# UWQuickstep/quickstep

Hardware: AMD Instinct MI355X
Metric: probe+aggregate rows/s at TPC-H SF100 (Q1,Q3) (higher is better)
Workload: dtype i32 keys / f64 sums

## Files before the change

### quickstep_amd/csrc/join.hip

```cpp

#include "common.hpp"
#include "join_dense.hpp"
#include "join_lds.hpp"
#include "scan.hpp"

#include <atomic>
#include <cstdlib>
#include <vector>
#include <mutex>
#include <shared_mutex>
#include <type_traits>

namespace qsx {

constexpr int kJBlock = 256;
constexpr uint64_t kEmpty64 = ~0ull;
constexpr uint32_t kEmptyTid = 0xFFFFFFFFu;

struct alignas(16) LongEntry {
  int64_t key;
  uint32_t tid;
  uint32_t pad;
};

// ... 1086 lines not shown
  if (rc_control != QSX_OK) return rc_control;
  t->reserved = 0;
  t->max_tid.store(-1);
  t->seal_state.store(0);
  t->scanned.store(false);
  drop_cover(t);
  mark_stream(t, as_stream(stream));
  return QSX_OK;
}

int qsx_join_table_size(qsx_join_table_t *t, int64_t *out_entries, qsx_stream_t stream) {
  QSX_REQUIRE_DEVICE();
  if (t == nullptr || out_entries == nullptr) return QSX_ERR_INVALID_ARGUMENT;
  unsigned long long v[kControlWords] = {0, 0, 0, 0, 0, 0};
  const int rc_words = copy_control_words(t->entries_dev, as_stream(stream), v);
  if (rc_words != QSX_OK) return rc_words;
  *out_entries = static_cast<int64_t>(v[0]);
  if (t->dense && static_cast<int>(v[3] & 0xFFFFFFFFu) != 0) return QSX_ERR_INVALID_ARGUMENT;
  return QSX_OK;
}

int qsx_join_build(qsx_join_table_t *t, const void *keys_dev, int64_t n, int32_t base_tid,
                   const uint64_t *filter_dev, qsx_stream_t stream) {
  QSX_REQUIRE_DEVICE();
  if (t == nullptr || n < 0 || base_tid < 0) return QSX_ERR_INVALID_ARGUMENT;
  if (n == 0) return QSX_OK;
  if (keys_dev == nullptr) return QSX_ERR_INVALID_ARGUMENT;
  if (static_cast<int64_t>(base_tid) + n > INT32_MAX) return QSX_ERR_INVALID_ARGUMENT;
  int rc = ensure_room(t, n);
  if (rc != QSX_OK) return rc;
  t->seal_state.store(0);
  t->scanned.store(false);
  drop_cover(t);
  for (int64_t seen = t->max_tid.load(); seen < base_tid + n - 1 && !t->max_tid.compare_exchange_weak(seen, base_tid + n - 1);) {}
  std::shared_lock<std::shared_mutex> lock(t->mutex);
  const int grid = grid_for(n, kJBlock * 4);
  if (t->dense) {
    const int dgrid = grid_for((n + 63) >> 6, (kDBlock / kWave) * kBuildR);
    if (t->key_type == QSX_INT) {
      hipLaunchKernelGGL(dense_build_kernel<int32_t>, dim3(dgrid), dim3(kDBlock), 0, as_stream(stream), t->dense_view(),
                         static_cast<const int32_t *>(keys_dev), n, base_tid, filter_dev, t->entries_dev);
    } else {
      hipLaunchKernelGGL(dense_build_kernel<int64_t>, dim3(dgrid), dim3(kDBlock), 0, as_stream(stream), t->dense_view(),
                         static_cast<const int64_t *>(keys_dev), n, base_tid, filter_dev, t->entries_dev);
    }
    QSX_CHECK_LAUNCH();
    return QSX_OK;
  }
  if (t->key_type == QSX_INT) {
    hipLaunchKernelGGL(build_kernel<int32_t>, dim3(grid), dim3(kJBlock), 0, as_stream(stream), t->view(),
                       static_cast<const int32_t *>(keys_dev), n, base_tid, filter_dev, t->entries_dev);
  } else {
    hipLaunchKernelGGL(build_kernel<int64_t>, dim3(grid), dim3(kJBlock), 0, as_stream(stream), t->view(),
                       static_cast<const int64_t *>(keys_dev), n, base_tid, filter_dev, t->entries_dev);
  }
  QSX_CHECK_LAUNCH();
  mark_stream(t, as_stream(stream));
  return QSX_OK;
}

static int check_key_coding(const qsx_key_coding_t **coding, int64_t num_blocks) {
  if (*coding == nullptr) return QSX_OK;
  if ((*coding)->block_code_width == nullptr) {
    *coding = nullptr;
    return QSX_OK;
  }
  bool any = false;
  for (int64_t b = 0; b < num_blocks; ++b) {
    const int w = (*coding)->block_code_width[b];
    if (w != 0 && w != 1 && w != 2 && w != 4) return QSX_ERR_INVALID_ARGUMENT;
    if (w == 0 && (*coding)->block_dictionaries != nullptr && (*coding)->block_dictionaries[b] != nullptr) return QSX_ERR_INVALID_ARGUMENT;
    any = any || w != 0;
  }
  if (!any) *coding = nullptr;
  return QSX_OK;
}

static int join_build_blocks_impl(qsx_join_table_t *t, int64_t num_blocks, const int64_t *block_rows, const void *const *block_keys,
                          const int32_t *block_base_tids, const uint64_t *const *block_filters, const qsx_key_coding_t *coding, qsx_stream_t stream) {
  QSX_REQUIRE_DEVICE();
  if (t == nullptr || num_blocks < 0 || (num_blocks > 0 && (block_rows == nullptr || block_keys == nullptr || block_base_tids == nullptr))) {
    return QSX_ERR_INVALID_ARGUMENT;
  }
  if (check_key_coding(&coding, num_blocks) != QSX_OK) return QSX_ERR_INVALID_ARGUMENT;
  std::vector<int64_t> base(static_cast<size_t>(num_blocks));
  int64_t total = 0;
  for (int64_t b = 0; b < num_blocks; ++b) {
    if (block_rows[b] < 0 || (block_rows[b] > 0 && block_keys[b] == nullptr) || block_base_tids[b] < 0 ||
        static_cast<int64_t>(block_base_tids[b]) + block_rows[b] > INT32_MAX) {
      return QSX_ERR_INVALID_ARGUMENT;
    }
    base[b] = block_base_tids[b];
    total += block_rows[b];
  }
  if (total == 0) return QSX_OK;
  int rc = ensure_room(t, total);
  if (rc != QSX_OK) return rc;
  t->seal_state.store(0);
  t->scanned.store(false);
  drop_cover(t);
  for (int64_t b = 0; b < num_blocks; ++b) {
    const int64_t last = base[b] + block_rows[b] - 1;
    for (int64_t seen = t->max_tid.load(); seen < last && !t->max_tid.compare_exchange_weak(seen, last);) {}
  }
  hipStream_t s = as_stream(stream);
  std::vector<long long> table;
  const long long groups = build_run_table(kBuildTile, num_blocks, block_rows, block_keys,
                                           reinterpret_cast<const void *const *>(block_filters), nullptr, base.data(), &table,
                                           coding != nullptr ? coding->block_code_width : nullptr,
                                           coding != nullptr ? coding->block_dictionaries : nullptr);
  if (groups < 0) return QSX_ERR_INVALID_ARGUMENT;
  const size_t bytes = table.size() * sizeof(long long);
  const long long *runs_dev = static_cast<const long long *>(staged_device_buffer(s, bytes));
  if (runs_dev == nullptr) return QSX_ERR_OUT_OF_MEMORY;
  rc = staged_upload(s, table.data(), bytes);
  if (rc != QSX_OK) return rc;
  std::shared_lock<std::shared_mutex> lock(t->mutex);
  if (t->dense) {
    const int dgrid = grid_for(groups, kDBlock / kWave);
    if (t->key_type == QSX_INT) {
      hipLaunchKernelGGL((dense_build_kernel<int32_t, true>), dim3(dgrid), dim3(kDBlock), 0, s, t->dense_view(),
                         static_cast<const int32_t *>(nullptr), total, 0, static_cast<const uint64_t *>(nullptr), t->entries_dev, runs_dev);
    } else {
      hipLaunchKernelGGL((dense_build_kernel<int64_t, true>), dim3(dgrid), dim3(kDBlock), 0, s, t->dense_view(),
                         static_cast<const int64_t *>(nullptr), total, 0, static_cast<const uint64_t *>(nullptr), t->entries_dev, runs_dev);
    }
  } else {
    const int grid = grid_for(groups, kJBlock / kWave);
    if (t->key_type == QSX_INT) {
      hipLaunchKernelGGL(build_runs_kernel<int32_t>, dim3(grid), dim3(kJBlock), 0, s, t->view(), runs_dev, t->entries_dev);
    } else {
      hipLaunchKernelGGL(build_runs_kernel<int64_t>, dim3(grid), dim3(kJBlock), 0, s, t->view(), runs_dev, t->entries_dev);
    }
  }
  QSX_CHECK_LAUNCH();
  mark_stream(t, s);
  return QSX_OK;
}

int qsx_join_build_blocks(qsx_join_table_t *t, int64_t num_blocks, const int64_t *block_rows, const void *const *block_keys,
                          const int32_t *block_base_tids, const uint64_t *const *block_filters, qsx_stream_t stream) {
  return join_build_blocks_impl(t, num_blocks, block_rows, block_keys, block_base_tids, block_filters, nullptr, stream);
}
int qsx_join_build_blocks_coded(qsx_join_table_t *t, int64_t num_blocks, const int64_t *block_rows, const void *const *block_keys,
                                const qsx_key_coding_t *coding, const int32_t *block_base_tids, const uint64_t *const *block_filters,
                                qsx_stream_t stream) {
  return join_build_blocks_impl(t, num_blocks, block_rows, block_keys, block_base_tids, block_filters, coding, stream);
}

}

static std::atomic<long long> g_compact_probes{0};
extern "C" long long qsx_debug_join_compact_probes(void) { return g_compact_probes.load(std::memory_order_relaxed); }
static bool lds_tables_enabled() {
  const char *e = getenv("QSX_JOIN_LDS");
  return e == nullptr || e[0] != '0';
}

static bool dense_two_pass(const uint64_t *filter) {
  const char *e = getenv("QSX_JOIN_TWO_PASS");
  if (e != nullptr && e[0] != '\0') return e[0] != '0';
  return filter != nullptr;
}

static void drop_cover(qsx_join_table *t) {
  std::lock_guard<std::mutex> lock(t->cover_mutex);
  t->cover_state = 0;
  t->cover_sig.clear();
}

constexpr int64_t kAdaptiveMinRows = 1 << 16;
static bool adaptive_enabled() {
  const char *e = getenv("QSX_JOIN_ADAPTIVE");
  return e == nullptr || e[0] != '0';
}

static void sealed_pack(qsx_join_table *t, hipStream_t stream) {
  auto behind_the_pack = [&]() {
    if (t->pack_stream != stream && t->pack_event != nullptr && hipEventQuery(t->pack_event) != hipSuccess) {
      (void)hipGetLastError();
      (void)hipStreamWaitEvent(stream, t->pack_event, 0);
    }
  };
  int state = t->seal_state.load(std::memory_order_acquire);
  if (state == 2) {
    behind_the_pack();
    return;
  }
  if (state != 0 || !adaptive_enabled()) return;
  const uint64_t bytes4 = t->range * 4, bytes3 = t->range * 3;
  if (bytes4 <= (13ull << 18) || bytes3 > (36ull << 20) / 10 || t->max_tid.load() >= (1 << 23) - 2 || t->reserved >= (1 << 23) - 1) {
    return;
  }
  std::lock_guard<std::mutex> lock(t->seal_mutex);
  state = t->seal_state.load(std::memory_order_acquire);
  if (state != 0) {
    if (state == 2) behind_the_pack();
    return;
  }
  if (t->head3 == nullptr && device_malloc(&t->head3, static_cast<size_t>(bytes3) + 4) != hipSuccess) {
    (void)hipGetLastError();
    t->head3 = nullptr;
    t->seal_state.store(1, std::memory_order_release);
    return;
  }
  if (t->pack_event == nullptr && hipEventCreateWithFlags(&t->pack_event, hipEventDisableTiming) != hipSuccess) {
    (void)hipGetLastError();
    t->pack_event = nullptr;
    t->seal_state.store(1, std::memory_order_release);
    return;
  }
  hipLaunchKernelGGL(dense_pack_kernel, dim3(grid_for(static_cast<int64_t>(t->range), kJBlock * 4)), dim3(kJBlock), 0, stream, t->head, t->range,
                     t->head3);
  if (hipGetLastError() != hipSuccess || hipEventRecord(t->pack_event, stream) != hipSuccess) {
    (void)hipGetLastError();
    (void)hipStreamSynchronize(stream);
    t->seal_state.store(1, std::memory_order_release);
    return;
  }
  t->pack_stream = stream;
  t->seal_state.store(2, std::memory_order_release);
}

static bool compact_enabled() {
  const char *e = getenv("QSX_JOIN_COMPACT");
  return e == nullptr || e[0] != '0';
}
static bool compact_possible(const qsx_join_table *t) {
  const uint64_t buckets = t->capacity / kBucketSlots;
  return compact_enabled() && t->key_type == QSX_INT && buckets >= kCompactMinBuckets && buckets <= 0xFFFFFFFFull && t->max_tid.load() < (1 << 24);
}
static bool seal_compact(qsx_join_table *t, bool duplicate_keys, hipStream_t stream) {
  if (!compact_possible(t) || duplicate_keys) return false;
  if (t->compact_capacity != t->capacity) {
    (void)device_free(t->compact);
    t->compact = nullptr;
    t->compact_capacity = 0;
    if (device_malloc(&t->compact, static_cast<size_t>(t->capacity) * 5 + 16) != hipSuccess) {
      (void)hipGetLastError();
      t->compact = nullptr;
      return false;
    }
    t->compact_capacity = t->capacity;
  }
  hipLaunchKernelGGL(compact_build_kernel, dim3(static_cast<unsigned>((t->capacity + kJBlock - 1) / kJBlock)), dim3(kJBlock), 0, stream, t->view(),
                     static_cast<uint32_t *>(t->compact), static_cast<unsigned char *>(t->compact) + t->capacity * 4);
  if (hipGetLastError() != hipSuccess) return false;
  return true;
}

static bool seal_verify_enabled() {
  const char *e = getenv("QSX_JOIN_SEAL_VERIFY");
  return e != nullptr && e[0] == '1';
}
static bool wait_for_builds(qsx_join_table *t, hipStream_t stream) {
  bool marked = true;
  std::lock_guard<std::mutex> lock(t->marks_mutex);
  for (const auto &m : t->marks) {
    if (m.second == nullptr) marked = false;
    else if (m.first != stream && hipStreamWaitEvent(stream, m.second, 0) != hipSuccess) marked = false;
  }
  if (!marked) (void)hipGetLastError();
  return marked;
}
static bool read_control_words(qsx_join_table *t, hipStream_t stream, unsigned long long *v, bool *any_key) {
  if (t->control_host == nullptr && hipHostMalloc(reinterpret_cast<void **>(&t->control_host), kControlBytes, hipHostMallocDefault) != hipSuccess) {
    (void)hipGetLastError();
    t->control_host = nullptr;
  }
  if (t->control_host == nullptr) return copy_control_words(t->entries_dev, stream, v, any_key) == QSX_OK;
  if (hipMemcpyAsync(t->control_host, t->entries_dev, kControlBytes, hipMemcpyDeviceToHost, stream) != hipSuccess ||
      hipStreamSynchronize(stream) != hipSuccess) {
    return false;
  }
  *any_key = fold_control_words(t->control_host, v);
  return true;
}
static void behind_the_seal(qsx_join_table *t, hipStream_t stream) {
  if (t->seal_stream != stream && t->seal_event != nullptr && hipEventQuery(t->seal_event) != hipSuccess) {
    (void)hipGetLastError();
    (void)hipStreamWaitEvent(stream, t->seal_event, 0);
  }
}
static bool record_seal(qsx_join_table *t, hipStream_t stream) {
  if (t->seal_event == nullptr && hipEventCreateWithFlags(&t->seal_event, hipEventDisableTiming) != hipSuccess) {
    (void)hipGetLastError();
    t->seal_event = nullptr;
  }
  if (t->seal_event == nullptr || hipEventRecord(t->seal_event, stream) != hipSuccess) {
    (void)hipGetLastError();
    if (hipStreamSynchronize(stream) != hipSuccess) return false;
    t->seal_stream = nullptr;
    if (t->seal_event != nullptr) {
      (void)hipEventDestroy(t->seal_event);
      t->seal_event = nullptr;
    }
  } else {
    t->seal_stream = stream;
  }
  return true;
}
static bool publish_seal(qsx_join_table *t, hipStream_t stream, int state) {
  if (!record_seal(t, stream)) return false;
  t->seal_state.store(state, std::memory_order_release);
  return true;
}
// ... 42 lines not shown
    return nullptr;
  };
  if (!adaptive_enabled()) return stays_hashed();
  if (not_worth_a_look) {
    (void)ensure_scanned();
    return nullptr;
  }
  unsigned long long v[kControlWords];
  bool any_key = false;
  if (!put_behind_builds() || !read_control_words(t, stream, v, &any_key)) return stays_hashed();
  const uint64_t entries = v[0];
  const int64_t lo = static_cast<int64_t>(v[4] ^ 0x8000000000000000ull), hi = static_cast<int64_t>(v[5] ^ 0x8000000000000000ull);
  const uint64_t span = static_cast<uint64_t>(hi) - static_cast<uint64_t>(lo);
  const bool fits_lds = small_build && entries >= 1 && span < static_cast<uint64_t>(kLdsDenseMaxWords);
  if (!any_key || (entries < static_cast<uint64_t>(kAdaptiveMinRows) && !fits_lds) || (span >= 8 * entries && !fits_lds) ||
      span >= (1ull << 32) || entries > 0x7FFFFFFFull) {
    if (!ensure_scanned()) return nullptr;
    if (!compact_possible(t) || !read_control_words(t, stream, v, &any_key) || !seal_compact(t, v[2] != 0, stream) || !publish_seal(t, stream, 3)) {
      t->seal_state.store(1, std::memory_order_release);
    }
    return nullptr;
  }
  qsx_join_table *shadow = t->shadow;
  if (shadow != nullptr && (shadow->min_key != lo || shadow->range != span + 1 || shadow->ov_capacity < entries)) {
    (void)qsx_join_table_destroy(shadow);
    shadow = t->shadow = nullptr;
  }
  if (shadow == nullptr) {
    if (qsx_join_table_create_dense(t->key_type, lo, hi, 1, static_cast<int64_t>(entries), &shadow) != QSX_OK) {
      (void)hipGetLastError();
      return stays_hashed();
    }
    t->shadow = shadow;
  } else if (qsx_join_table_clear(shadow, reinterpret_cast<qsx_stream_t>(stream)) != QSX_OK) {
    return stays_hashed();
  }
  shadow->reserved = static_cast<int64_t>(entries);
  shadow->max_tid.store(t->max_tid.load());
  const TableView src = t->view();
  hipLaunchKernelGGL(dense_build_from_slots_kernel, dim3(grid_for(static_cast<int64_t>(src.num_slots()), kJBlock * 4)), dim3(kJBlock), 0, stream,
                     t->key_type == QSX_LONG ? 1 : 0, src, shadow->dense_view());
  if (hipGetLastError() != hipSuccess) return stays_hashed();
  if (seal_verify_enabled()) {
    int error = 0;
    if (hipStreamSynchronize(stream) != hipSuccess ||
        hipMemcpy(&error, shadow->entries_dev + 3, sizeof(error), hipMemcpyDeviceToHost) != hipSuccess || error != 0) {
      set_last_error("QSX_JOIN_SEAL_VERIFY: the shadow's build reported an error", hipErrorUnknown);
      return stays_hashed();
    }
  }
  if (!publish_seal(t, stream, 2)) return stays_hashed();
  return shadow;
}

template <int MODE, bool kRuns, bool kLds = true, int NLIP = 0>
static int launch_lds_dense_probe(qsx_join_table_t *t, const void *keys, int64_t n, int32_t probe_base_tid, const uint64_t *filter,
                                  int32_t *out_probe, int32_t *out_build, int64_t capacity, unsigned long long *count,
                                  uint64_t *out_bitmap, int anti, hipStream_t stream, const long long *runs_dev, int64_t tiles,
                                  const LipViews &lips = LipViews{}) {
  const size_t table_bytes = kLds ? ((static_cast<size_t>(t->range) * 4 + 15) & ~static_cast<size_t>(15)) : 0;
  auto launch = [&](auto key_tag) -> int {
    using KeyT = decltype(key_tag);
    auto kernel = &lds_dense_probe_kernel<KeyT, MODE, kRuns, kLds, NLIP>;
    if (table_bytes > 48 * 1024) {
      QSX_HIP_TRY(hipFuncSetAttribute(reinterpret_cast<const void *>(kernel), hipFuncAttributeMaxDynamicSharedMemorySize, 160 * 1024 - kLdsStaticBytes));
    }
    const int sub = kLds ? kLdsSub : kLdsSubGlobal, per_cu = kLds ? 1 : 2;
    const int64_t units = (tiles + sub - 1) / sub;
    const int grid = static_cast<int>(units < static_cast<int64_t>(per_cu) * kCUs ? units : static_cast<int64_t>(per_cu) * kCUs);
    hipLaunchKernelGGL(kernel, dim3(grid), dim3(kLdsBlock), table_bytes, stream, t->dense_view(), static_cast<const KeyT *>(keys), n, probe_base_tid,
                       filter, out_probe, out_build, capacity, count, out_bitmap, anti, runs_dev, lips);
    QSX_CHECK_LAUNCH();
    return QSX_OK;
  };
  return t->key_type == QSX_INT ? launch(int32_t{}) : launch(int64_t{});
}

static bool one_pass_enabled() {
  const char *e = getenv("QSX_JOIN_ONE_PASS");
  return e == nullptr || e[0] != '0';
}

template <int MODE, bool kRuns = false>
static int launch_probe(qsx_join_table_t *t, const void *keys, int64_t n, int32_t probe_base_tid,
                        const uint64_t *filter, int32_t *out_probe, int32_t *out_build,
                        int64_t capacity, int64_t *out_count, uint64_t *out_bitmap, int anti,
                        hipStream_t stream, const long long *runs_dev = nullptr, int64_t run_tiles = 0) {
  static_assert(kDenseTile == kProbeTile, "one run table serves both table kinds");
  if (!t->dense && n != 0) {
    qsx_join_table *shadow = sealed_shadow(t, stream, n);
    if (shadow != nullptr) {
      return launch_probe<MODE, kRuns>(shadow, keys, n, probe_base_tid, filter, out_probe, out_build, capacity, out_count, out_bitmap,
                                       anti, stream, runs_dev, run_tiles);
    }
    if (!t->scanned.load(std::memory_order_acquire)) {
      set_last_error("the scan in front of a hashed table's first probe could not be issued", hipErrorUnknown);
      return QSX_ERR_HIP;
    }
  }
  if (out_count != nullptr) QSX_HIP_TRY(hipMemsetAsync(out_count, 0, sizeof(int64_t), stream));
  if (n == 0) return QSX_OK;
  if (t->dense) sealed_pack(t, stream);
  std::shared_lock<std::shared_mutex> lock(t->mutex);
  if (t->dense) {
    const int64_t tiles = kRuns ? run_tiles : (n + kDenseTile - 1) / kDenseTile;
    const int64_t limit = 8 * kCUs;
    const int dgrid = static_cast<int>(tiles < limit ? tiles : limit);
    unsigned long long *dcount = reinterpret_cast<unsigned long long *>(out_count);
    if constexpr (MODE == 0 || MODE == 1 || MODE == 2) {
      const bool two_pass = MODE == 0 && dense_two_pass(filter);
      if (!two_pass && lds_tables_enabled() && t->range <= static_cast<uint64_t>(kLdsDenseMaxWords) && n >= 32 * static_cast<int64_t>(t->range) &&
          n >= (1 << 18)) {
        return launch_lds_dense_probe<MODE, kRuns>(t, keys, n, probe_base_tid, filter, out_probe, out_build, capacity, dcount, out_bitmap, anti,
                                                   stream, runs_dev, tiles);
      }
    }
    if constexpr (MODE == 0) {
      if (dense_two_pass(filter) && one_pass_enabled() && n >= (1 << 20)) {
        return launch_lds_dense_probe<0, kRuns, false>(t, keys, n, probe_base_tid, filter, out_probe, out_build, capacity, dcount, out_bitmap, anti,
                                                       stream, runs_dev, tiles);
      }
    }
    if (MODE == 0 && dense_two_pass(filter)) {
      const int64_t units = tiles * (kDBlock / kWave);
      CallScratch scratch(stream);
      const size_t bytes_counts = static_cast<size_t>(units) * 4, bytes_offsets = static_cast<size_t>(units + 1) * 8,
                   bytes_scan = scan_workspace_words(units) * 8;
      const int rc_scratch = scratch.reserve(CallScratch::padded(bytes_counts) + CallScratch::padded(bytes_offsets) + CallScratch::padded(bytes_scan));
      if (rc_scratch != QSX_OK) return rc_scratch;
      int32_t *unit_counts = static_cast<int32_t *>(scratch.take(bytes_counts));
      int64_t *unit_offsets = static_cast<int64_t *>(scratch.take(bytes_offsets)), *scan_ws = static_cast<int64_t *>(scratch.take(bytes_scan));
      if (t->key_type == QSX_INT) {
        hipLaunchKernelGGL((dense_probe_kernel<int32_t, 3, kRuns>), dim3(dgrid), dim3(kDBlock), 0, stream, t->dense_view(),
                           static_cast<const int32_t *>(keys), n, probe_base_tid, filter, out_probe, out_build, capacity,
                           dcount, out_bitmap, anti, unit_counts, unit_offsets, runs_dev);
      } else {
        hipLaunchKernelGGL((dense_probe_kernel<int64_t, 3, kRuns>), dim3(dgrid), dim3(kDBlock), 0, stream, t->dense_view(),
                           static_cast<const int64_t *>(keys), n, probe_base_tid, filter, out_probe, out_build, capacity,
                           dcount, out_bitmap, anti, unit_counts, unit_offsets, runs_dev);
      }
      QSX_CHECK_LAUNCH();
      QSX_HIP_TRY(launch_scan(unit_counts, units, unit_offsets, out_count, scan_ws, stream));
      if (t->key_type == QSX_INT) {
        hipLaunchKernelGGL((dense_probe_kernel<int32_t, 4, kRuns>), dim3(dgrid), dim3(kDBlock), 0, stream, t->dense_view(),
                           static_cast<const int32_t *>(keys), n, probe_base_tid, filter, out_probe, out_build, capacity,
                           dcount, out_bitmap, anti, unit_counts, unit_offsets, runs_dev);
      } else {
        hipLaunchKernelGGL((dense_probe_kernel<int64_t, 4, kRuns>), dim3(dgrid), dim3(kDBlock), 0, stream, t->dense_view(),
                           static_cast<const int64_t *>(keys), n, probe_base_tid, filter, out_probe, out_build, capacity,
                           dcount, out_bitmap, anti, unit_counts, unit_offsets, runs_dev);
      }
      QSX_CHECK_LAUNCH();
      return QSX_OK;
    }
    if (t->key_type == QSX_INT) {
      hipLaunchKernelGGL((dense_probe_kernel<int32_t, MODE, kRuns>), dim3(dgrid), dim3(kDBlock), 0, stream, t->dense_view(),
                         static_cast<const int32_t *>(keys), n, probe_base_tid, filter, out_probe, out_build, capacity,
                         dcount, out_bitmap, anti, nullptr, nullptr, runs_dev);
    } else {
      hipLaunchKernelGGL((dense_probe_kernel<int64_t, MODE, kRuns>), dim3(dgrid), dim3(kDBlock), 0, stream, t->dense_view(),
                         static_cast<const int64_t *>(keys), n, probe_base_tid, filter, out_probe, out_build, capacity,
                         dcount, out_bitmap, anti, nullptr, nullptr, runs_dev);
    }
    QSX_CHECK_LAUNCH();
    return QSX_OK;
  }
  const int64_t num_tiles = kRuns ? run_tiles : (n + kProbeTile - 1) / kProbeTile;
  if constexpr (MODE == 0 || MODE == 1 || MODE == 2) {
    if (lds_tables_enabled() && t->table_bytes() <= kLdsBucketMaxBytes && n >= (1 << 18) && n >= 8 * static_cast<int64_t>(t->capacity)) {
      const size_t table_bytes = (t->table_bytes() + 15) & ~static_cast<size_t>(15);
      auto launch = [&](auto key_tag) -> int {
        using KeyT = decltype(key_tag);
        auto kernel = &lds_bucket_probe_kernel<KeyT, MODE, kRuns>;
        if (table_bytes > 48 * 1024) {
          QSX_HIP_TRY(hipFuncSetAttribute(reinterpret_cast<const void *>(kernel), hipFuncAttributeMaxDynamicSharedMemorySize, 160 * 1024 - kLdsStaticBytes));
        }
        const int64_t units = (num_tiles + kLdsSub - 1) / kLdsSub;
        const int lgrid = static_cast<int>(units < kCUs ? units : kCUs);
        hipLaunchKernelGGL(kernel, dim3(lgrid), dim3(kLdsBlock), table_bytes, stream, t->view(), static_cast<const KeyT *>(keys), n, probe_base_tid, filter,
                           out_probe, out_build, capacity, reinterpret_cast<unsigned long long *>(out_count), out_bitmap, anti, runs_dev);
        QSX_CHECK_LAUNCH();
        return QSX_OK;
      };
      return t->key_type == QSX_INT ? launch(int32_t{}) : launch(int64_t{});
    }
  }
  const int64_t max_grid = MODE == 0 ? 4 * kCUs : 8 * kCUs;
  const int grid = static_cast<int>(num_tiles < max_grid ? num_tiles : max_grid);
  unsigned long long *count = reinterpret_cast<unsigned long long *>(out_count);
  if constexpr (MODE == 0 || MODE == 1 || MODE == 2) {
    if (t->key_type == QSX_INT && t->seal_state.load(std::memory_order_acquire) == 3 && compact_enabled()) {
      g_compact_probes.fetch_add(1, std::memory_order_relaxed);
      hipLaunchKernelGGL((probe_fp_kernel<int32_t, MODE, kRuns, true>), dim3(grid), dim3(kJBlock), 0, stream, t->view(),
                         static_cast<const int32_t *>(keys), n, probe_base_tid, filter, out_probe,
                         out_build, capacity, count, out_bitmap, anti, runs_dev, t->compact_view());
      QSX_CHECK_LAUNCH();
      return QSX_OK;
    }
  }
  if (t->key_type == QSX_INT) {
    hipLaunchKernelGGL((probe_fp_kernel<int32_t, MODE, kRuns>), dim3(grid), dim3(kJBlock), 0, stream, t->view(),
                       static_cast<const int32_t *>(keys), n, probe_base_tid, filter, out_probe,
                       out_build, capacity, count, out_bitmap, anti, runs_dev);
  } else {
    hipLaunchKernelGGL((probe_fp_kernel<int64_t, MODE, kRuns>), dim3(grid), dim3(kJBlock), 0, stream, t->view(),
                       static_cast<const int64_t *>(keys), n, probe_base_tid, filter, out_probe,
                       out_build, capacity, count, out_bitmap, anti, runs_dev);
  }
  QSX_CHECK_LAUNCH();
  return QSX_OK;
}

static int cover_for(qsx_join_table *t, const ProjectionView &view, int entry_bytes, bool wanted, const std::vector<long long> &signature,
                     hipStream_t stream, const void **cover) {
  const char *env = getenv("QSX_JOIN_COVER");
  if (!wanted || entry_bytes <= 0 || (env != nullptr && env[0] == '0') || !adaptive_enabled()) return 0;
  std::lock_guard<std::mutex> lock(t->cover_mutex);
  if (t->cover_state != 0 && t->cover_sig == signature) {
    *cover = t->cover;
    return t->cover_state == 2 ? t->cover_entry_bytes : 0;
  }
  if (t->cover_state == 2 && hipDeviceSynchronize() != hipSuccess) return 0;
  t->cover_state = 1;
  t->cover_sig = signature;
  const size_t bytes = static_cast<size_t>(t->range) * entry_bytes;
  if (bytes > (size_t(1) << 30)) return 0;
  if (t->cover_bytes < bytes) {
    (void)device_free(t->cover);
    t->cover = nullptr;
    t->cover_bytes = 0;
    if (device_malloc(&t->cover, bytes + 16) != hipSuccess) {
      (void)hipGetLastError();
      t->cover = nullptr;
      return 0;
    }
    t->cover_bytes = bytes;
  }
  unsigned int *flags = reinterpret_cast<unsigned int *>(static_cast<char *>(t->cover) + bytes);
  if (hipMemsetAsync(flags, 0, sizeof(unsigned int), stream) != hipSuccess) return 0;
  const DenseTableView dv = t->dense_view();
  const unsigned grid = static_cast<unsigned>((t->range + kDBlock - 1) / kDBlock);
  switch (entry_bytes) {
    case 4: hipLaunchKernelGGL(cover_build_kernel<uint32_t>, dim3(grid), dim3(kDBlock), 0, stream, dv, view, static_cast<uint32_t *>(t->cover), flags); break;
    case 8: hipLaunchKernelGGL(cover_build_kernel<unsigned long long>, dim3(grid), dim3(kDBlock), 0, stream, dv, view,
                               static_cast<unsigned long long *>(t->cover), flags); break;
    default: hipLaunchKernelGGL(cover_build_kernel<ulonglong2>, dim3(grid), dim3(kDBlock), 0, stream, dv, view, static_cast<ulonglong2 *>(t->cover), flags); break;
  }
  unsigned int seen = 0;
  if (hipGetLastError() != hipSuccess || hipStreamSynchronize(stream) != hipSuccess ||
      hipMemcpy(&seen, flags, sizeof(seen), hipMemcpyDeviceToHost) != hipSuccess || seen != 0) {
    (void)hipGetLastError();
    return 0;
  }
  t->cover_entry_bytes = entry_bytes;
  t->cover_state = 2;
  *cover = t->cover;
  return entry_bytes;
}

static int upload_probe_run(int64_t num_blocks, const int64_t *block_rows, const void *const *block_keys,
                            const int32_t *block_base_tids, const uint64_t *const *block_filters, uint64_t *const *block_out,
                            hipStream_t stream, const long long **runs_dev, int64_t *tiles, int64_t *rows_total, bool *any_filter,
                            const std::vector<long long> *extra = nullptr, const long long **extra_dev = nullptr,
                            const qsx_key_coding_t *coding = nullptr) {
  std::vector<int64_t> base(static_cast<size_t>(num_blocks));
  int64_t total = 0;
  *any_filter = false;
  for (int64_t b = 0; b < num_blocks; ++b) {
    if (block_rows[b] < 0 || (block_rows[b] > 0 && block_keys[b] == nullptr)) return QSX_ERR_INVALID_ARGUMENT;
    if (block_rows[b] > 0 && block_out != nullptr && block_out[b] == nullptr) return QSX_ERR_INVALID_ARGUMENT;
    base[b] = block_base_tids != nullptr ? block_base_tids[b] : total;
    if (base[b] < 0 || base[b] + block_rows[b] > INT32_MAX) return QSX_ERR_INVALID_ARGUMENT;
    total += block_rows[b];
    if (block_filters != nullptr && block_filters[b] != nullptr) *any_filter = true;
  }
  std::vector<long long> table;
  *tiles = build_run_table(kDenseTile, num_blocks, block_rows, block_keys, reinterpret_cast<const void *const *>(block_filters),
                           reinterpret_cast<void *const *>(block_out), base.data(), &table,
                           coding != nullptr ? coding->block_code_width : nullptr, coding != nullptr ? coding->block_dictionaries : nullptr);
  *rows_total = total;
  if (*tiles < 0) return QSX_ERR_INVALID_ARGUMENT;
  if (*tiles == 0) return QSX_OK;
  const size_t run_words = table.size();
  if (extra != nullptr) table.insert(table.end(), extra->begin(), extra->end());
  const size_t bytes = table.size() * sizeof(long long);
  *runs_dev = static_cast<const long long *>(staged_device_buffer(stream, bytes));
  if (*runs_dev == nullptr) return QSX_ERR_OUT_OF_MEMORY;
  if (extra_dev != nullptr) *extra_dev = *runs_dev + run_words;
  return staged_upload(stream, table.data(), bytes);
}

namespace qsx {
constexpr int kLipFromTableWords = kWave;
__global__ __launch_bounds__(256) void lip_from_dense_kernel(DenseTableView t, LipView f, long long delta, long long first_word,
                                                             long long end_word) {
  const int lane = lane_id();
  const long long wave = static_cast<long long>(blockIdx.x) * (256 / kWave) + (threadIdx.x >> 6);
  const long long num_waves = static_cast<long long>(gridDim.x) * (256 / kWave);
  for (long long w0 = first_word + wave * kLipFromTableWords; w0 < end_word; w0 += num_waves * kLipFromTableWords) {
    unsigned long long mine = 0ull;
#pragma unroll
    for (int r0 = 0; r0 < kLipFromTableWords; r0 += 8) {
      uint32_t head[8];
#pragma unroll
      for (int u = 0; u < 8; ++u) {
        const long long word = w0 + r0 + u;
// ... 426 lines not shown
```

### quickstep_amd/csrc/join_dense.hpp

```cpp
#ifndef QSX_CSRC_JOIN_DENSE_HPP_
#define QSX_CSRC_JOIN_DENSE_HPP_

#include <type_traits>

#include "block_runs.hpp"
#include "common.hpp"

namespace qsx {

constexpr int kDBlock = 256;
constexpr int kDenseRowsPerThread = 16;
constexpr int kDenseTile = kDBlock * kDenseRowsPerThread;
constexpr uint32_t kChainBit = 0x80000000u;
constexpr int kDenseSparsePairs = 256;

struct DenseTableView {
  uint32_t *head;
  const unsigned char *head3;
  uint2 *ov;
  int64_t min_key;
  int stride_shift;
  uint64_t range;
  unsigned int *ov_count;
  unsigned int ov_capacity;
// ... 70 lines not shown
    const int32_t base_tid = cur.base_tid;
    cur = next;
    uint64_t idx[R];
    uint32_t old[R];
#pragma unroll
    for (int r = 0; r < R; ++r) {
      const int64_t i = ((w0 + r) << 6) + lane;
      const uint64_t fw = __shfl(words, r, kWave);
      const bool live = i < n && msb_bit(fw, lane);
      idx[r] = live ? dense_index(t, key[r]) : ~1ull;
      if (idx[r] == ~0ull) atomicExch(t.error, 1);
      old[r] = 0u;
      if (idx[r] < ~1ull) old[r] = atomicCAS(&t.head[idx[r]], 0u, static_cast<uint32_t>(base_tid + i) + 1u);
    }
#pragma unroll
    for (int r = 0; r < R; ++r) {
      if (idx[r] >= ~1ull) continue;
      const int64_t i = ((w0 + r) << 6) + lane;
      const uint32_t tid = static_cast<uint32_t>(base_tid + i);
      if (old[r] != 0u) {
        const unsigned int e = atomicAdd(t.ov_count, 1u);
        if (e >= t.ov_capacity) {
          atomicExch(t.error, 2);
          continue;
        }
        t.ov[e].x = tid;
        t.ov[e].y = atomicExch(&t.head[idx[r]], kChainBit | e);
      }
      ++inserted;
    }
#pragma unroll
    for (int r = 0; r < R; ++r) key[r] = next_key[r];
    words = next_words;
  }
  inserted = wave_reduce_add(inserted);
  if (lane == 0 && inserted != 0) atomicAdd(entries + static_cast<size_t>(wave & 31) * 16, inserted);
}

constexpr int kProjColumnWords = 5;
struct ProjectionView {
  const long long *table;
  int nc;
  int nseg;
  int seg_rows;
  const void *cover;
  __device__ __forceinline__ int width(int c) const { return static_cast<int>(table[c]); }
  __device__ __forceinline__ bool on_build(int c) const { return table[nc + c] != 0; }
  __device__ __forceinline__ char *out(int c) const { return as_global(reinterpret_cast<char *>(table[2 * nc + c])); }
  __device__ __forceinline__ int cover_offset(int c) const { return static_cast<int>(table[3 * nc + c]); }
  __device__ __forceinline__ bool is_probe_key(int c) const { return table[4 * nc + c] != 0; }
  __device__ __forceinline__ const long long *first_tids() const { return table + kProjColumnWords * nc; }
  __device__ __forceinline__ const char *build_stripe(int seg, int c) const {
    return as_global(reinterpret_cast<const char *>(table[kProjColumnWords * nc + nseg + seg * nc + c]));
  }
  __device__ __forceinline__ const char *probe_stripe(int block, int c) const {
    return as_global(reinterpret_cast<const char *>(table[kProjColumnWords * nc + nseg + nseg * nc + block * nc + c]));
  }
};
__device__ __forceinline__ unsigned long long load_value(const char *src, int width) {
  switch (width) {
    case 1: return load_global(reinterpret_cast<const uint8_t *>(src));
    case 2: return load_global(reinterpret_cast<const uint16_t *>(src));
    case 4: return load_global(reinterpret_cast<const uint32_t *>(src));
    default: return load_global(reinterpret_cast<const unsigned long long *>(src));
  }
}
__device__ __forceinline__ void store_value(char *dst, unsigned long long v, int width) {
  switch (width) {
    case 1: store_global(static_cast<uint8_t>(v), reinterpret_cast<uint8_t *>(dst)); break;
    case 2: store_global(static_cast<uint16_t>(v), reinterpret_cast<uint16_t *>(dst)); break;
    case 4: store_global_nt(static_cast<uint32_t>(v), reinterpret_cast<uint32_t *>(dst)); break;
    default: store_global_nt(v, reinterpret_cast<unsigned long long *>(dst)); break;
  }
}
__device__ __forceinline__ const char *projected_build_value(const ProjectionView &p, int c, int width, uint32_t tid) {
  const long long *first = p.first_tids();
  int seg = 0;
  if (p.nseg > 1) {
    if (p.seg_rows > 0) {
      seg = static_cast<int>((tid - static_cast<uint32_t>(first[0])) / static_cast<uint32_t>(p.seg_rows));
      seg = seg < p.nseg ? seg : p.nseg - 1;
    } else {
      int lo = 0, hi = p.nseg - 1;
      while (lo < hi) {
        const int mid = (lo + hi + 1) >> 1;
        if (first[mid] <= static_cast<long long>(tid)) lo = mid; else hi = mid - 1;
      }
      seg = lo;
    }
  }
  return p.build_stripe(seg, c) + static_cast<size_t>(tid - static_cast<uint32_t>(first[seg])) * width;
}
template <typename KeyT>
__device__ __forceinline__ void project_one(const ProjectionView &p, const ProbeTileSource<KeyT> &tile, int64_t probe_row, uint32_t tid,
                                            unsigned long long o) {
  for (int c = 0; c < p.nc; ++c) {
    const int width = p.width(c);
    if (!p.on_build(c) && tile.code_width != 0 && p.is_probe_key(c)) {
      store_value(p.out(c) + o * width, static_cast<unsigned long long>(coded_key(tile, probe_row)), width);
      continue;
    }
    const char *src = p.on_build(c) ? projected_build_value(p, c, width, tid) : p.probe_stripe(tile.block, c) + static_cast<size_t>(probe_row) * width;
    store_value(p.out(c) + o * width, load_value(src, width), width);
  }
}

template <typename EntryT>
__global__ __launch_bounds__(kDBlock) void cover_build_kernel(DenseTableView t, ProjectionView p, EntryT *__restrict__ cover,
                                                             unsigned int *__restrict__ flags) {
  const uint64_t i = static_cast<uint64_t>(blockIdx.x) * kDBlock + threadIdx.x;
  if (i >= t.range) return;
  const uint32_t hw = t.head[i];
  unsigned long long words[2] = {~0ull, ~0ull};
  if (hw & kChainBit) {
    atomicOr(flags, 1u);
  } else if (hw != 0u) {
    words[0] = words[1] = 0ull;
    for (int c = 0; c < p.nc; ++c) {
      if (!p.on_build(c)) continue;
      const int width = p.width(c), off = p.cover_offset(c);
      const unsigned long long v = load_value(projected_build_value(p, c, width, hw - 1u), width);
      if (off < 8) words[0] |= v << (8 * off); else words[1] |= v << (8 * (off - 8));
    }
    const bool ones = sizeof(EntryT) == 4 ? static_cast<uint32_t>(words[0]) == ~0u
                                          : (sizeof(EntryT) == 8 ? words[0] == ~0ull : (words[0] & words[1]) == ~0ull);
    if (ones) atomicOr(flags, 2u);
  }
  if constexpr (sizeof(EntryT) == 4) {
    cover[i] = static_cast<uint32_t>(words[0]);
  } else if constexpr (sizeof(EntryT) == 8) {
    cover[i] = words[0];
  } else {
    cover[i] = EntryT{words[0], words[1]};
  }
}

__device__ __forceinline__ void dense_emit_direct(bool match, int32_t probe_tid, int32_t build_tid,
                                                  int32_t *__restrict__ out_probe, int32_t *__restrict__ out_build,
                                                  unsigned long long capacity, unsigned long long *out_count) {
  const uint64_t m = __ballot(match);
  if (m == 0) return;
  unsigned long long base = 0;
  if (lane_id() == __ffsll(static_cast<long long>(m)) - 1) {
    base = atomicAdd(out_count, static_cast<unsigned long long>(__popcll(m)));
  }
  base = __shfl(base, __ffsll(static_cast<long long>(m)) - 1, kWave);
  const unsigned long long o = base + rank_below(m);
  if (match && o < capacity) {
    __builtin_nontemporal_store(probe_tid, &out_probe[o]);
    __builtin_nontemporal_store(build_tid, &out_build[o]);
  }
}

template <typename KeyT, int MODE, bool kRuns = false>
__global__ __launch_bounds__(kDBlock) __attribute__((amdgpu_waves_per_eu(MODE == 5 ? 3 : 1))) void dense_probe_kernel(
    DenseTableView t, const KeyT *__restrict__ keys, int64_t n, int32_t probe_base_tid,
    const uint64_t *__restrict__ filter, int32_t *__restrict__ out_probe, int32_t *__restrict__ out_build,
    int64_t capacity_signed, unsigned long long *__restrict__ out_count, uint64_t *__restrict__ out_bitmap, int anti,
    int32_t *__restrict__ unit_counts = nullptr, const int64_t *__restrict__ unit_offsets = nullptr,
    const long long *__restrict__ runs = nullptr, ProjectionView proj = ProjectionView{}) {
  constexpr int R = kDenseRowsPerThread;
  constexpr bool kProject = MODE == 5;
  using Source = ProbeTileSource<KeyT>;
  const unsigned long long capacity = static_cast<unsigned long long>(capacity_signed);
  const int64_t num_tiles = kRuns ? runs[2] : (n + kDenseTile - 1) / kDenseTile;
  auto source_of = [&](int64_t tile) {
    return probe_tile_source<KeyT, kDenseTile, kRuns>(runs, tile, keys, n, probe_base_tid, filter, out_bitmap);
  };
  unsigned long long local_count = 0;
  __shared__ int2 s_sparse[(MODE == 0 || MODE == 4) ? kDBlock / kWave : 1][(MODE == 0 || MODE == 4) ? kDenseSparsePairs : 1];
  __shared__ int s_wave_total[2][kDBlock / kWave];
  __shared__ unsigned long long s_tile_base;
  int parity = 0;
  const int wave = threadIdx.x >> 6;

  const int lane = lane_id();
  KeyT key[R], next_key[R];
  uint64_t filter_words = ~0ull, next_filter_words = ~0ull;
  auto request = [&](const Source &src, KeyT (&k)[R], uint64_t &words) {
    if (kRuns && src.code_width != 0) {
      coded_keys(src, k, [&](int r) {
        const int64_t row = src.base + r * kDBlock + threadIdx.x;
        return row < src.n ? row : src.n - 1;
      });
    } else {
#pragma unroll
      for (int r = 0; r < R; ++r) {
        const int64_t row = src.base + r * kDBlock + threadIdx.x;
        k[r] = load_global_nt(&src.keys[row < src.n ? row : src.n - 1]);
      }
    }
    words = ~0ull;
    if (src.filter != nullptr && lane < R) {
      const int64_t w = (src.base >> 6) + lane * (kDBlock / kWave) + wave;
      if (w < ((src.n + 63) >> 6)) words = load_global(&src.filter[w]);
    }
  };
  Source cur = Source(), next = Source();
  if (static_cast<int64_t>(blockIdx.x) < num_tiles) {
    cur = source_of(blockIdx.x);
    request(cur, key, filter_words);
  }

  for (int64_t tile = blockIdx.x; tile < num_tiles; tile += gridDim.x, parity ^= 1) {
    if (tile + gridDim.x < num_tiles) {
      next = source_of(tile + gridDim.x);
      request(next, next_key, next_filter_words);
    }
    const int64_t tile_base = cur.base;
    const int64_t n_rows = cur.n;
    const int32_t base_tid = cur.base_tid;
    uint64_t *const tile_bitmap = cur.out_bitmap;
    const int tile_block = cur.block;
    const Source tile_src = cur;
    cur = next;
    uint32_t h[R];
    uint32_t live_mask = 0;
#pragma unroll
    for (int r = 0; r < R; ++r) {
      const int64_t row = tile_base + r * kDBlock + threadIdx.x;
      const uint64_t filter_word = __shfl(filter_words, r, kWave);
      const bool live = row < n_rows && msb_bit(filter_word, lane);
      live_mask |= live ? (1u << r) : 0u;
      const uint64_t idx = dense_index(t, key[r]);
      const bool lookup = live && idx != ~0ull;
      const uint32_t word = dense_head_word(t, lookup ? idx : 0);
      h[r] = lookup ? word : 0u;
    }
#pragma unroll
    for (int r = 0; r < R; ++r) key[r] = next_key[r];
    filter_words = next_filter_words;

    if (MODE == 2) {
      uint64_t mine = 0;
#pragma unroll
      for (int r = 0; r < R; ++r) {
        const bool bit = ((live_mask >> r) & 1u) && ((h[r] != 0u) != (anti != 0));
        const uint64_t word = msb_first(__ballot(bit));
        if (lane == r) mine = word;
        if (lane == 0) local_count += __popcll(word);
      }
      const int64_t w = (tile_base >> 6) + lane * (kDBlock / kWave) + wave;
      if (lane < R && w < ((n_rows + 63) >> 6)) store_global(mine, &tile_bitmap[w]);
      continue;
    }

    uint64_t m[R];
    int total = 0;
    bool any_chain = false;
#pragma unroll
    for (int r = 0; r < R; ++r) {
      m[r] = __ballot(h[r] != 0u);
      total += __popcll(m[r]);
      any_chain = any_chain || (h[r] & kChainBit) != 0u;
    }
    const bool wave_has_chain = __any(any_chain);
    uint32_t next[R];
    unsigned long long base = 0;
    if (MODE == 1 || MODE == 3) {
      if (lane == 0) local_count += total;
      if (wave_has_chain) {
#pragma unroll
        for (int r = 0; r < R; ++r) next[r] = (h[r] & kChainBit) ? t.ov[h[r] & ~kChainBit].y : 0u;
      }
    } else {
      if (MODE == 0 || kProject) {
        if (lane == 0) s_wave_total[parity][wave] = total;
        __syncthreads();
        if (threadIdx.x == 0) {
          int all = 0;
#pragma unroll
          for (int w = 0; w < kDBlock / kWave; ++w) all += s_wave_total[parity][w];
          s_tile_base = all != 0 ? atomicAdd(out_count, static_cast<unsigned long long>(all)) : 0ull;
        }
        __syncthreads();
        base = s_tile_base;
        for (int w = 0; w < wave; ++w) base += s_wave_total[parity][w];
      } else {
        base = static_cast<unsigned long long>(unit_offsets[tile * (kDBlock / kWave) + wave]);
      }
      const bool sparse = !kProject && total <= kDenseSparsePairs;
      int staged = 0;
      if (kProject) {
        int off[R];
        int emitted = 0;
#pragma unroll
        for (int r = 0; r < R; ++r) {
          next[r] = 0u;
          if (wave_has_chain && (h[r] & kChainBit)) {
            const uint2 e = t.ov[h[r] & ~kChainBit];
            h[r] = e.x + 1u;
            next[r] = e.y;
          }
          off[r] = emitted + rank_below(m[r]);
          emitted += __popcll(m[r]);
        }
        const unsigned long long wave_base = base;
        base += emitted;
        for (int c = 0; c < proj.nc; ++c) {
          const int width = proj.width(c);
          const bool on_build = proj.on_build(c);
          char *dst = proj.out(c);
          const char *probe_stripe = proj.probe_stripe(tile_block, c);
          auto column = [&](auto tag) __attribute__((always_inline)) {
            using V = decltype(tag);
            constexpr int H = R / 2;
#pragma unroll
            for (int half = 0; half < 2; ++half) {
              V v[H];
              if (on_build) {
#pragma unroll
                for (int i = 0; i < H; ++i) {
                  const int r = half * H + i;
                  const char *src = h[r] != 0u ? projected_build_value(proj, c, sizeof(V), h[r] - 1u) : dst;
                  v[i] = load_global(reinterpret_cast<const V *>(src));
                }
              } else if (kRuns && sizeof(V) == sizeof(KeyT) && tile_src.code_width != 0 && proj.is_probe_key(c)) {
#pragma unroll
                for (int i = 0; i < H; ++i) {
                  const int64_t row = tile_base + (half * H + i) * kDBlock + threadIdx.x;
                  v[i] = static_cast<V>(coded_key(tile_src, row < n_rows ? row : n_rows - 1));
                }
              } else {
#pragma unroll
                for (int i = 0; i < H; ++i) {
                  const int64_t row = tile_base + (half * H + i) * kDBlock + threadIdx.x;
                  v[i] = load_global_nt(&reinterpret_cast<const V *>(probe_stripe)[row < n_rows ? row : n_rows - 1]);
                }
              }
#pragma unroll
              for (int i = 0; i < H; ++i) {
                const int r = half * H + i;
                const unsigned long long o = wave_base + off[r];
                if (h[r] != 0u && o < capacity) store_global_nt(v[i], reinterpret_cast<V *>(dst) + o);
              }
            }
          };
          switch (width) {
            case 1: column(uint8_t{}); break;
            case 2: column(uint16_t{}); break;
            case 4: column(uint32_t{}); break;
            default: column(static_cast<unsigned long long>(0)); break;
          }
        }
      }
#pragma unroll
      for (int r = 0; r < R; ++r) {
        if (kProject) break;
        const int64_t row = tile_base + r * kDBlock + threadIdx.x;
        uint32_t tid = h[r] - 1u;
        next[r] = 0u;
        if (wave_has_chain && (h[r] & kChainBit)) {
          const uint2 e = t.ov[h[r] & ~kChainBit];
          tid = e.x;
          next[r] = e.y;
        }
        if (sparse) {
          if (m[r] != 0) {
            if (h[r] != 0u) s_sparse[wave][staged + rank_below(m[r])] = make_int2(static_cast<int32_t>(base_tid + row), static_cast<int32_t>(tid));
            staged += __popcll(m[r]);
          }
        } else {
          const unsigned long long o = base + rank_below(m[r]);
          if (h[r] != 0u && o < capacity) {
            __builtin_nontemporal_store(static_cast<int32_t>(base_tid + row), &out_probe[o]);
            __builtin_nontemporal_store(static_cast<int32_t>(tid), &out_build[o]);
          }
          base += __popcll(m[r]);
        }
      }
      if (sparse) {
        __builtin_amdgcn_fence(__ATOMIC_RELEASE, "wavefront");
        __builtin_amdgcn_wave_barrier();
        __builtin_amdgcn_fence(__ATOMIC_ACQUIRE, "wavefront");
        for (int i = lane; i < total; i += kWave) {
          const int2 pair = s_sparse[wave][i];
          const unsigned long long o = base + i;
          if (o < capacity) {
            __builtin_nontemporal_store(pair.x, &out_probe[o]);
            __builtin_nontemporal_store(pair.y, &out_build[o]);
          }
        }
        base += total;
        __builtin_amdgcn_wave_barrier();
      }
    }
    if (wave_has_chain) {
#pragma unroll 1
      for (int r = 0; r < R; ++r) {
        const int64_t row = tile_base + r * kDBlock + threadIdx.x;
        uint32_t cur = next[r];
        while (__any(cur != 0u)) {
          uint32_t tid = cur - 1u, nxt = 0u;
          if (cur & kChainBit) {
            const uint2 e = t.ov[cur & ~kChainBit];
            tid = e.x;
            nxt = e.y;
          }
          if (MODE == 1 || MODE == 3) {
            local_count += cur != 0u ? 1u : 0u;
          } else if (MODE == 0) {
            dense_emit_direct(cur != 0u, static_cast<int32_t>(base_tid + row), static_cast<int32_t>(tid), out_probe,
                              out_build, capacity, out_count);
          } else if (kProject) {
            const uint64_t cm = __ballot(cur != 0u);
            unsigned long long at = 0;
            const int leader = __ffsll(static_cast<long long>(cm)) - 1;
            if (lane == leader) at = atomicAdd(out_count, static_cast<unsigned long long>(__popcll(cm)));
            at = __shfl(at, leader, kWave) + rank_below(cm);
            if (cur != 0u && at < capacity) project_one(proj, tile_src, row, tid, at);
          } else {
            const uint64_t cm = __ballot(cur != 0u);
            const unsigned long long o = base + rank_below(cm);
            if (cur != 0u && o < capacity) {
              __builtin_nontemporal_store(static_cast<int32_t>(base_tid + row), &out_probe[o]);
              __builtin_nontemporal_store(static_cast<int32_t>(tid), &out_build[o]);
            }
            base += __popcll(cm);
          }
          cur = nxt;
        }
      }
    }
    if (MODE == 3) {
      const unsigned long long unit = wave_reduce_add(local_count);
      if (lane == 0) unit_counts[tile * (kDBlock / kWave) + wave] = static_cast<int32_t>(unit);
      local_count = 0;
    }
  }
  if (MODE == 1 || MODE == 2) {
    local_count = wave_reduce_add(local_count);
    if (lane == 0 && local_count != 0 && out_count != nullptr) atomicAdd(out_count, local_count);
  }
}

template <typename KeyT, typename CoverT, int BLOCK>
__global__ __launch_bounds__(BLOCK) void cover_probe_kernel(DenseTableView t, int64_t capacity_signed,
                                                             unsigned long long *__restrict__ out_count,
                                                             const long long *__restrict__ runs, ProjectionView proj) {
  constexpr int R = kDenseTile / BLOCK;
  static_assert(R * BLOCK == kDenseTile && R <= kWave, "a tile is R steps of BLOCK rows; lane r holds the filter word of step r");
  const unsigned long long capacity = static_cast<unsigned long long>(capacity_signed);
  const int64_t num_tiles = runs[2];
  __shared__ int s_wave_total[2][BLOCK / kWave];
  __shared__ unsigned long long s_tile_base;
  const int wave = threadIdx.x >> 6, lane = lane_id();
  const CoverT *cover = reinterpret_cast<const CoverT *>(proj.cover);
  int parity = 0;
  for (int64_t tile = blockIdx.x; tile < num_tiles; tile += gridDim.x, parity ^= 1) {
    const ProbeTileSource<KeyT> src = probe_tile_source<KeyT, kDenseTile, true>(runs, tile, nullptr, 0, 0, nullptr, nullptr);
    uint64_t filter_words = ~0ull;
    if (src.filter != nullptr && lane < R) {
      const int64_t w = (src.base >> 6) + lane * (BLOCK / kWave) + wave;
      if (w < ((src.n + 63) >> 6)) filter_words = load_global(&src.filter[w]);
    }
    CoverT e[R];
    KeyT key[R];
    {
      if (src.code_width != 0) {
        coded_keys(src, key, [&](int r) {
          const int64_t row = src.base + r * BLOCK + threadIdx.x;
          return row < src.n ? row : src.n - 1;
        });
      } else {
#pragma unroll
        for (int r = 0; r < R; ++r) {
          const int64_t row = src.base + r * BLOCK + threadIdx.x;
          key[r] = load_global_nt(&src.keys[row < src.n ? row : src.n - 1]);
        }
      }
#pragma unroll
      for (int r = 0; r < R; ++r) {
        const uint64_t idx = dense_index(t, key[r]);
        if constexpr (sizeof(CoverT) == 16) {
          using Pair = unsigned long long __attribute__((ext_vector_type(2)));
          const Pair both = load_global(reinterpret_cast<const Pair *>(&cover[idx != ~0ull ? idx : 0]));
          e[r] = CoverT{both.x, both.y};
        } else {
          e[r] = load_global(&cover[idx != ~0ull ? idx : 0]);
        }
        if (idx == ~0ull) {
          if constexpr (sizeof(CoverT) == 16) e[r] = CoverT{~0ull, ~0ull}; else e[r] = static_cast<CoverT>(~static_cast<CoverT>(0));
        }
      }
    }
    uint64_t m[R];
    int total = 0;
#pragma unroll
    for (int r = 0; r < R; ++r) {
      const int64_t row = src.base + r * BLOCK + threadIdx.x;
      const uint64_t filter_word = __shfl(filter_words, r, kWave);
      bool present;
      if constexpr (sizeof(CoverT) == 16) present = (e[r].x & e[r].y) != ~0ull; else present = e[r] != static_cast<CoverT>(~static_cast<CoverT>(0));
      m[r] = __ballot(present && row < src.n && msb_bit(filter_word, lane));
      total += __popcll(m[r]);
    }
    if (lane == 0) s_wave_total[parity][wave] = total;
    __syncthreads();
    if (threadIdx.x == 0) {
      int all = 0;
#pragma unroll
      for (int w = 0; w < BLOCK / kWave; ++w) all += s_wave_total[parity][w];
      s_tile_base = all != 0 ? atomicAdd(out_count, static_cast<unsigned long long>(all)) : 0ull;
    }
    __syncthreads();
    unsigned long long base = s_tile_base;
    for (int w = 0; w < wave; ++w) base += s_wave_total[parity][w];
    if (total == 0) continue;
    int off[R];
    unsigned int emit_mask = 0;
    {
      int at = 0;
#pragma unroll
      for (int r = 0; r < R; ++r) {
        off[r] = at + rank_below(m[r]);
        if (((m[r] >> lane) & 1ull) && base + static_cast<unsigned long long>(off[r]) < capacity) emit_mask |= 1u << r;
        at += __popcll(m[r]);
      }
    }
    const int tile_rows = static_cast<int>(src.n - src.base < kDenseTile ? src.n - src.base : kDenseTile);
    for (int c = 0; c < proj.nc; ++c) {
      const int width = proj.width(c);
      const bool on_build = proj.on_build(c);
      const int shift = 8 * proj.cover_offset(c);
      const bool from_key = proj.is_probe_key(c);
      auto column = [&](auto tag) __attribute__((always_inline)) {
        using V = decltype(tag);
        constexpr int H = R / 2;
        V *tile_dst = reinterpret_cast<V *>(proj.out(c)) + base;
        const V *tile_src = reinterpret_cast<const V *>(proj.probe_stripe(src.block, c)) + src.base;
#pragma unroll
        for (int half = 0; half < 2; ++half) {
          V v[H];
#pragma unroll
          for (int i = 0; i < H; ++i) {
            const int r = half * H + i;
            if (on_build) {
              if constexpr (sizeof(CoverT) == 16) {
                v[i] = static_cast<V>(shift < 64 ? e[r].x >> shift : e[r].y >> (shift - 64));
              } else {
                v[i] = static_cast<V>(static_cast<unsigned long long>(e[r]) >> shift);
              }
            } else if (from_key && sizeof(V) == sizeof(KeyT)) {
// ... 27 lines not shown
```

Baseline: 190.5 billion.

## Add wide-vector row mapping for unfiltered dense join probe loads and pair stores

Adds a kWide variant of the dense probe kernel for the plain pair-emitting mode without a filter. Each thread now owns kPer consecutive rows, so keys can be read with 16-byte nontemporal vector loads. When a group of four rows fully matches, has no chains and the output base is aligned, the output pairs are written as 16-byte vector stores. This is meant to cut the number of memory instructions on the key reads and pair writes. In exchange it adds per-group ballot checks and makes the output order within a wave differ from the scalar mapping.

```diff
diff --git a/quickstep_amd/csrc/join.hip b/quickstep_amd/csrc/join.hip
--- a/quickstep_amd/csrc/join.hip
+++ b/quickstep_amd/csrc/join.hip
@@ -1262,6 +1262,12 @@
 
 static std::atomic<long long> g_compact_probes{0};
 extern "C" long long qsx_debug_join_compact_probes(void) { return g_compact_probes.load(std::memory_order_relaxed); }
+static std::atomic<long long> g_wide_probes{0};
+extern "C" long long qsx_debug_join_wide_probes(void) { return g_wide_probes.load(std::memory_order_relaxed); }
+static bool wide_probe_enabled() {
+  const char *e = getenv("QSX_JOIN_WIDE");
+  return e == nullptr || e[0] != '0';
+}
 static bool lds_tables_enabled() {
   const char *e = getenv("QSX_JOIN_LDS");
   return e == nullptr || e[0] != '0';
@@ -1610,6 +1616,22 @@
       }
       QSX_CHECK_LAUNCH();
       return QSX_OK;
+    }
+    if constexpr (MODE == 0 && !kRuns) {
+      if (filter == nullptr && (reinterpret_cast<uintptr_t>(keys) & 15u) == 0 && n >= kDenseTile && wide_probe_enabled()) {
+        g_wide_probes.fetch_add(1, std::memory_order_relaxed);
+        if (t->key_type == QSX_INT) {
+          hipLaunchKernelGGL((dense_probe_kernel<int32_t, 0, false, true>), dim3(dgrid), dim3(kDBlock), 0, stream, t->dense_view(),
+                             static_cast<const int32_t *>(keys), n, probe_base_tid, filter, out_probe, out_build, capacity,
+                             dcount, out_bitmap, anti, nullptr, nullptr, runs_dev);
+        } else {
+          hipLaunchKernelGGL((dense_probe_kernel<int64_t, 0, false, true>), dim3(dgrid), dim3(kDBlock), 0, stream, t->dense_view(),
+                             static_cast<const int64_t *>(keys), n, probe_base_tid, filter, out_probe, out_build, capacity,
+                             dcount, out_bitmap, anti, nullptr, nullptr, runs_dev);
+        }
+        QSX_CHECK_LAUNCH();
+        return QSX_OK;
+      }
     }
     if (t->key_type == QSX_INT) {
       hipLaunchKernelGGL((dense_probe_kernel<int32_t, MODE, kRuns>), dim3(dgrid), dim3(kDBlock), 0, stream, t->dense_view(),
diff --git a/quickstep_amd/csrc/join_dense.hpp b/quickstep_amd/csrc/join_dense.hpp
--- a/quickstep_amd/csrc/join_dense.hpp
+++ b/quickstep_amd/csrc/join_dense.hpp
@@ -246,7 +246,7 @@
   }
 }
 
-template <typename KeyT, int MODE, bool kRuns = false>
+template <typename KeyT, int MODE, bool kRuns = false, bool kWide = false>
 __global__ __launch_bounds__(kDBlock) __attribute__((amdgpu_waves_per_eu(MODE == 5 ? 3 : 1))) void dense_probe_kernel(
     DenseTableView t, const KeyT *__restrict__ keys, int64_t n, int32_t probe_base_tid,
     const uint64_t *__restrict__ filter, int32_t *__restrict__ out_probe, int32_t *__restrict__ out_build,
@@ -255,6 +255,17 @@
     const long long *__restrict__ runs = nullptr, ProjectionView proj = ProjectionView{}) {
   constexpr int R = kDenseRowsPerThread;
   constexpr bool kProject = MODE == 5;
+  static_assert(!kWide || (MODE == 0 && !kRuns), "the wide row mapping exists for the plain pair-emitting form only");
+  constexpr int kPer = 16 / static_cast<int>(sizeof(KeyT));
+  typedef KeyT WideKeys __attribute__((ext_vector_type(kPer)));
+  typedef int32_t WidePairs __attribute__((ext_vector_type(4)));
+  auto row_of = [&](int64_t tile_base, int r, [[maybe_unused]] bool wide) __attribute__((always_inline)) -> int64_t {
+    if constexpr (kWide) {
+      if (wide) return tile_base + (r / kPer) * (kDBlock * kPer) + (r % kPer) + kPer * threadIdx.x;
+    }
+    return tile_base + r * kDBlock + threadIdx.x;
+  };
+  const bool wide_stores = kWide && ((reinterpret_cast<uintptr_t>(out_probe) | reinterpret_cast<uintptr_t>(out_build)) & 15u) == 0;
   using Source = ProbeTileSource<KeyT>;
   const unsigned long long capacity = static_cast<unsigned long long>(capacity_signed);
   const int64_t num_tiles = kRuns ? runs[2] : (n + kDenseTile - 1) / kDenseTile;
@@ -277,6 +288,14 @@
         const int64_t row = src.base + r * kDBlock + threadIdx.x;
         return row < src.n ? row : src.n - 1;
       });
+    } else if (kWide && src.base + kDenseTile <= src.n) {
+#pragma unroll
+      for (int s = 0; s < R / kPer; ++s) {
+        const WideKeys v = __builtin_nontemporal_load(
+            (const __attribute__((address_space(1))) WideKeys *)reinterpret_cast<uintptr_t>(src.keys + row_of(src.base, s * kPer, true)));
+#pragma unroll
+        for (int j = 0; j < kPer; ++j) k[s * kPer + j] = v[j];
+      }
     } else {
 #pragma unroll
       for (int r = 0; r < R; ++r) {
@@ -307,12 +326,13 @@
     uint64_t *const tile_bitmap = cur.out_bitmap;
     const int tile_block = cur.block;
     const Source tile_src = cur;
+    const bool wide_tile = kWide && tile_base + kDenseTile <= n_rows;
     cur = next;
     uint32_t h[R];
     uint32_t live_mask = 0;
 #pragma unroll
     for (int r = 0; r < R; ++r) {
-      const int64_t row = tile_base + r * kDBlock + threadIdx.x;
+      const int64_t row = row_of(tile_base, r, wide_tile);
       const uint64_t filter_word = __shfl(filter_words, r, kWave);
       const bool live = row < n_rows && msb_bit(filter_word, lane);
       live_mask |= live ? (1u << r) : 0u;
@@ -375,6 +395,7 @@
       }
       const bool sparse = !kProject && total <= kDenseSparsePairs;
       int staged = 0;
+      [[maybe_unused]] bool group_done = false;
       if (kProject) {
         int off[R];
         int emitted = 0;
@@ -441,7 +462,29 @@
 #pragma unroll
       for (int r = 0; r < R; ++r) {
         if (kProject) break;
-        const int64_t row = tile_base + r * kDBlock + threadIdx.x;
+        if constexpr (kWide) {
+          if ((r & 3) == 0) {
+            group_done = wide_tile && wide_stores && !sparse && (m[r] & m[r + 1] & m[r + 2] & m[r + 3]) == ~0ull && (base & 3u) == 0 &&
+                    base + 4 * kWave <= capacity &&
+                    !(wave_has_chain && __any(((h[r] | h[r + 1] | h[r + 2] | h[r + 3]) & kChainBit) != 0u));
+            if (group_done) {
+              const int32_t first = static_cast<int32_t>(base_tid + row_of(tile_base, r, true));
+              WidePairs rows, tids;
+#pragma unroll
+              for (int j = 0; j < 4; ++j) {
+                rows[j] = first + static_cast<int32_t>(row_of(0, r + j, true) - row_of(0, r, true));
+                tids[j] = static_cast<int32_t>(h[r + j] - 1u);
+                next[r + j] = 0u;
+              }
+              const unsigned long long o = base + 4u * static_cast<unsigned>(lane);
+              __builtin_nontemporal_store(rows, (__attribute__((address_space(1))) WidePairs *)reinterpret_cast<uintptr_t>(out_probe + o));
+              __builtin_nontemporal_store(tids, (__attribute__((address_space(1))) WidePairs *)reinterpret_cast<uintptr_t>(out_build + o));
+              base += 4 * kWave;
+            }
+          }
+          if (group_done) continue;
+        }
+        const int64_t row = row_of(tile_base, r, wide_tile);
         uint32_t tid = h[r] - 1u;
         next[r] = 0u;
         if (wave_has_chain && (h[r] & kChainBit)) {
@@ -482,7 +525,7 @@
     if (wave_has_chain) {
 #pragma unroll 1
       for (int r = 0; r < R; ++r) {
-        const int64_t row = tile_base + r * kDBlock + threadIdx.x;
+        const int64_t row = row_of(tile_base, r, wide_tile);
         uint32_t cur = next[r];
         while (__any(cur != 0u)) {
           uint32_t tid = cur - 1u, nxt = 0u;
```

Result: no change. 189.0 billion (-0.8%).
